# TalShor/SciLMM

Measured on NVIDIA B200. Metric: reml_iter_time, lower is better.
Workload: dtype f64

## Files before the change

### scilmm_b200/csrc/chol.cu

```cuda
#include <algorithm>
#include <cmath>
#include <cstring>
#include <map>
#include <memory>
#include <vector>

#include "common.h"
#include "dense_tiles.cuh"
#include "dense_tiles_tma.cuh"
#include "potrf_block.cuh"
#include "skinny_ops.cuh"
#include "symbolic.h"

namespace slmm {

static thread_local std::string g_last_error;
void set_last_error(const std::string& msg) { g_last_error = msg; }
const std::string& last_error() { return g_last_error; }
int64_t g_launch_count = 0;

constexpr int NBO = 1024;

struct PullItem { int32_t p, c0, c1, e0, e1; };
struct PullEntry { int64_t rel_off, src_off; int32_t rsc, ta, tb, pad; };
// ... 169 lines not shown

__global__ void logdet_kernel(const double* __restrict__ Lx, const int32_t* __restrict__ col2sn,
                              const int32_t* __restrict__ sn_first, const int32_t* __restrict__ sn_nrow,
                              const int64_t* __restrict__ sn_lptr, int n, double* __restrict__ partial) {
  __shared__ double sh[256];
  double acc = 0.0;
  for (int j = blockIdx.x * blockDim.x + threadIdx.x; j < n; j += gridDim.x * blockDim.x) {
    const int s = col2sn[j], c = j - sn_first[s];
    acc += log(Lx[sn_lptr[s] + (int64_t)c * ((sn_nrow[s] + 1) & ~1) + c]);
  }
  sh[threadIdx.x] = acc;
  __syncthreads();
  for (int o = 128; o > 0; o >>= 1) {
    if (threadIdx.x < o) sh[threadIdx.x] += sh[threadIdx.x + o];
    __syncthreads();
  }
  if (threadIdx.x == 0) partial[blockIdx.x] = sh[0];
}

struct Launch {
  enum Kind { POTRF, GEMM_BIG, GEMM_SMALL, PULL_MAT, PULL_VEC, PULL_MAT_BIG, INIT_W, REDUCE, EV_RECORD, EV_WAIT,
              SKINNY_F1, SKINNY_F2 ,
              GEMM_TMA  } kind;
  int64_t off;
  int32_t count;
  int32_t grid;
  int32_t child_parity;
  double flops;
  int64_t tile_off;
  int32_t stream;
  int64_t aux_off = 0;
};

static CUtensorMap encode_tmap(const double* base, uint64_t rows, uint64_t cols, uint64_t ld) {
  typedef CUresult (*EncodeFn)(CUtensorMap*, CUtensorMapDataType, cuuint32_t, void*, const cuuint64_t*, const cuuint64_t*,
                               const cuuint32_t*, const cuuint32_t*, CUtensorMapInterleave, CUtensorMapSwizzle,
                               CUtensorMapL2promotion, CUtensorMapFloatOOBfill);
  static EncodeFn fn = nullptr;
  if (!fn) {
    void* p = nullptr;
    cudaDriverEntryPointQueryResult q;
    CUDA_OK(cudaGetDriverEntryPoint("cuTensorMapEncodeTiled", &p, cudaEnableDefault, &q));
    if (!p || q != cudaDriverEntryPointSuccess) throw std::runtime_error("cuTensorMapEncodeTiled is not available");
    fn = (EncodeFn)p;
  }
  CUtensorMap m;
  const cuuint64_t gdim[2] = {rows, cols};
  const cuuint64_t gstride[1] = {ld * sizeof(double)};
  const cuuint32_t box[2] = {16, (cuuint32_t)TMA_KS};
  const cuuint32_t estr[2] = {1, 1};
  const CUresult rc = fn(&m, CU_TENSOR_MAP_DATA_TYPE_FLOAT64, 2, (void*)base, gdim, gstride, box, estr, CU_TENSOR_MAP_INTERLEAVE_NONE,
                         CU_TENSOR_MAP_SWIZZLE_128B, CU_TENSOR_MAP_L2_PROMOTION_L2_128B, CU_TENSOR_MAP_FLOAT_OOB_FILL_NONE);
  if (rc != CUDA_SUCCESS) throw std::runtime_error("cuTensorMapEncodeTiled failed (" + std::to_string((int)rc) + ")");
  return m;
}

constexpr int BIG_STAGES = 4, SMALL_STAGES = 4;
constexpr int BIG_SMEM = BIG_STAGES * 16 * (128 + 4) * 2 * 8 + 2 * BIG_STAGES * 8;
constexpr int SMALL_SMEM = SMALL_STAGES * 16 * (64 + 4) * 2 * 8 + 2 * SMALL_STAGES * 8;
constexpr int BIG_THREADS = 32 * (2 * 4 + NPW), SMALL_THREADS = 32 * (2 * 2 + NPW);

struct Schedule {
  std::vector<Launch> launches;
  std::vector<GemmOp> gemm;
  std::vector<PotrfOp> potrf;
  std::vector<PullItem> pull;
  std::vector<PullEntry> pull_entries;
  DevPtr<PullEntry> d_pull_entries;
  std::vector<ReduceOp> reduce;
  std::vector<CUtensorMap> tmaps;
  DevPtr<CUtensorMap> d_tmaps;
  std::vector<int32_t> tile_op;
  DevPtr<int32_t> d_tile_op;
  int nevents = 0;
  int64_t ws_size = 0;
  int64_t ws2_size = 0;
  DevPtr<double> d_ws;
  DevPtr<double> d_ws2;
  DevPtr<ReduceOp> d_reduce;
  DevPtr<GemmOp> d_gemm;
  DevPtr<PotrfOp> d_potrf;
  DevPtr<PullItem> d_pull;
  double flops = 0;
  GraphExec gexec[2];
  bool graph_failed = false;
  void upload() {
    if (ws_size > 0 || ws2_size > 0) {
      d_ws = dev_alloc<double>(ws_size);
      d_ws2 = dev_alloc<double>(ws2_size);
      for (GemmOp& op : gemm) {
        if (op.flags & GF_WS) { op.C = d_ws.get() + (int64_t)(intptr_t)op.C; op.flags &= ~GF_WS; }
        if (op.flags & GF_WS2) { op.C = d_ws2.get() + (int64_t)(intptr_t)op.C; op.flags &= ~GF_WS2; }
      }
      for (ReduceOp& r : reduce) {
        r.ws = ((r.flags & GF_WS2) ? d_ws2 : d_ws).get() + (int64_t)(intptr_t)r.ws;
        r.flags &= ~GF_WS2;
      }
    }
    d_reduce = dev_upload(reduce.data(), reduce.size());
    d_gemm = dev_upload(gemm.data(), gemm.size());
    d_potrf = dev_upload(potrf.data(), potrf.size());
    d_pull = dev_upload(pull.data(), pull.size());
    d_tile_op = dev_upload(tile_op.data(), tile_op.size());
    d_tmaps = dev_upload(tmaps.data(), tmaps.size());
    d_pull_entries = dev_upload(pull_entries.data(), pull_entries.size());
  }
  size_t device_bytes() const {
    return gemm.size() * sizeof(GemmOp) + potrf.size() * sizeof(PotrfOp) + pull.size() * sizeof(PullItem) +
           reduce.size() * sizeof(ReduceOp) + (size_t)(ws_size + ws2_size) * 8 + tile_op.size() * 4 + pull_entries.size() * sizeof(PullEntry);
  }
};

struct PhaseBuilder {
  std::vector<GemmOp> big, small, sk1, sk2;
  std::vector<GemmOp> tma;
  int skinny_mt = 0;
  int ws_id = 0;
  std::vector<PotrfOp> potrf;
  std::vector<ReduceOp> reduces;
  int64_t ws_used = 0;
  bool allow_split = true;
  static bool tma_ok(const GemmOp& op) {
    return op.a_si == 1 && op.b_sj == 1 && op.a_kidx == nullptr && !(op.flags & GF_TRIL_B) &&
           (op.a_sk % 2) == 0 && (op.b_sk % 2) == 0 && op.a_sk > 0 && op.b_sk > 0 && op.K >= 64;
  }
  void push(const GemmOp& op, bool small_tiles) {
    const bool tma_splits_inplace = op.C == op.A && op.N + (int)(((uintptr_t)op.B >> 3) & 1) > 128;
    if (small_tiles) small.push_back(op);
    else if (tma_ok(op) && !tma_splits_inplace) tma.push_back(op);
    else big.push_back(op);
  }
  template <typename Push>
  void split_k(const GemmOp& op, int S, int kc, Push push) {
    const int64_t mn = (int64_t)op.M * op.N;
    ReduceOp r;
    memset(&r, 0, sizeof(r));
    r.C = op.C; r.c_si = op.c_si; r.c_sj = op.c_sj; r.M = op.M; r.N = op.N; r.S = S;
    r.flags = (op.flags & (GF_ACCUM | GF_NEG)) | (ws_id ? GF_WS2 : 0);
    r.ws = (const double*)(intptr_t)ws_used;
    reduces.push_back(r);
    for (int c = 0; c < S; c++) {
      GemmOp part = op;
      const int k0 = c * kc;
      part.K = std::min(kc, op.K - k0);
      if (op.a_kidx) part.a_kidx = op.a_kidx + k0; else part.A = op.A + (int64_t)k0 * op.a_sk;
      part.B = op.B + (int64_t)k0 * op.b_sk;
      part.C = (double*)(intptr_t)(ws_used + (int64_t)c * mn);
      part.c_si = 1; part.c_sj = op.M;
      part.flags = (ws_id ? GF_WS2 : GF_WS) | (op.flags & GF_TRIL_B);
      part.pad = k0;
      push(part);
    }
    ws_used += (int64_t)S * mn;
  }
  bool add_skinny(const GemmOp& op) {
    if (skinny_mt <= 0 || op.M > skinny_mt || op.a_si != 1 || op.c_si != 1 || (op.flags & (GF_LOWER | GF_BIGTILE))) return false;
    const bool f1 = op.b_sj == 1 && op.a_kidx == nullptr;
    if (!f1 && op.b_sk != 1) return false;
    if (!f1 && (op.flags & GF_TRIL_B)) return false;
    std::vector<GemmOp>& dst = f1 ? sk1 : sk2;
    const int cols = f1 ? SK_F1_COLS : SK_F2_COLS, kmin = 64;
    const int64_t nj = (op.N + cols - 1) / cols;
    int S = 1;
    const int64_t target = f1 ? 148 * 8 : 148 * 4;
    const bool can_split = allow_split && op.C != op.A;
    if (can_split && nj < target) S = (int)std::min<int64_t>((target + nj - 1) / nj, std::max(1, op.K / kmin));
    if (!f1 && skinny_mt < 8) S = std::max(S, (op.K + SK_F2_KMAX - 1) / SK_F2_KMAX);
    if (S > 1 && !can_split) return false;
    int kc = op.K;
    if (S > 1) {
      kc = (((op.K + S - 1) / S) + 15) / 16 * 16;
      if (!f1 && skinny_mt < 8) kc = std::min(kc, SK_F2_KMAX);
      S = (op.K + kc - 1) / kc;
    }
    if (S <= 1) { GemmOp o = op; o.pad = 0; dst.push_back(o); }
    else split_k(op, S, kc, [&](const GemmOp& part) { dst.push_back(part); });
    return true;
  }
  void add(GemmOp op) {
    if (op.M <= 0 || op.N <= 0 || op.K <= 0) return;
    if (add_skinny(op)) return;
    const bool lower = op.flags & GF_LOWER;
    const int64_t tb = (int64_t)((op.M + 127) / 128) * ((op.N + 127) / 128);
    const int64_t ts = (int64_t)((op.M + 63) / 64) * ((op.N + 63) / 64);
    const bool force_big = op.flags & GF_BIGTILE;
    op.flags &= ~GF_BIGTILE;
    const bool small_tiles = !force_big && (!(op.M > 64 && op.N > 64) || (!lower && tb < 40 && op.K >= 128) ||
                                            (lower && tb <= 64));
    const int64_t tiles = small_tiles ? ts : tb;
    if (allow_split && !lower && (op.flags & GF_TRIL_B) && op.K >= 4096 && op.C != op.A && !small_tiles) {
      const int kc = 2048;
      const int S = (op.K + kc - 1) / kc;
      split_k(op, S, kc, [&](GemmOp part) { part.flags = (ws_id ? GF_WS2 : GF_WS) | GF_TRIL_B; push(part, false); });
      return;
    }
    if (allow_split && !lower && !(op.flags & GF_TRIL_B) && tiles <= 148 && op.K >= 256 && op.C != op.A) {
      int S = (int)std::min<int64_t>(std::min<int64_t>(64, op.K / 64), std::max<int64_t>(1, 148 / tiles));
      const int kc = S > 0 ? (((op.K + S - 1) / S) + 15) / 16 * 16 : op.K;
      S = (op.K + kc - 1) / kc;
      if (S >= 2) {
        op.flags &= ~GF_TRIL_B;
        split_k(op, S, kc, [&](GemmOp part) { part.pad = 0; part.flags = ws_id ? GF_WS2 : GF_WS; push(part, small_tiles); });
        return;
      }
    }
    push(op, small_tiles);
  }
  void flush(Schedule& sch, int stream = 0) {
    const size_t first_launch = sch.launches.size();
    if (!potrf.empty()) {
      double pf = 0;
      for (const PotrfOp& o : potrf) pf += 2.0 * o.nb * o.nb * o.nb / 3.0;
      sch.launches.push_back({Launch::POTRF, (int64_t)sch.potrf.size(), (int32_t)potrf.size(), (int32_t)potrf.size(), 0, pf});
      sch.potrf.insert(sch.potrf.end(), potrf.begin(), potrf.end());
    }
    for (int pass = 0; pass < 3; pass++) {
      std::vector<GemmOp>& v = pass == 0 ? tma : pass == 1 ? big : small;
      if (v.empty()) continue;
      const int T = pass == 2 ? 64 : 128;
      int64_t tiles = 0;
      double lf = 0;
      for (GemmOp& op : v) {
        int em = 0, en = 0;
        if (pass == 0) {
          em = (int)(((uintptr_t)op.A >> 3) & 1);
          en = (int)(((uintptr_t)op.B >> 3) & 1);
          op.pad = em | (en << 1);
        }
        op.tiles_m = (op.M + em + T - 1) / T;
        op.tiles_n = (op.N + en + T - 1) / T;
        op.tile_start = (int32_t)tiles;
        tiles += (int64_t)op.tiles_m * op.tiles_n;
        double f = 2.0 * op.M * op.N * op.K;
        if (op.flags & GF_TRIL_B) f = (double)op.M * op.N * op.K;
        if (op.flags & GF_LOWER) {
          const double nn = std::min(op.M, op.N);
          f = 2.0 * op.K * ((double)op.M * op.N - nn * (nn - 1) / 2.0);
        }
        sch.flops += f;
        lf += f;
      }
      if (tiles > 2000000000LL) throw std::runtime_error("too many tiles in one phase");
      const int64_t tile_off = (int64_t)sch.tile_op.size();
      sch.tile_op.resize(tile_off + tiles);
      for (size_t q = 0; q < v.size(); q++)
        std::fill(sch.tile_op.begin() + tile_off + v[q].tile_start,
                  sch.tile_op.begin() + tile_off + v[q].tile_start + (int64_t)v[q].tiles_m * v[q].tiles_n, (int32_t)q);
      if (pass == 0) {
        for (GemmOp& op : v) {
          const int sa = op.pad & 1, sb = (op.pad >> 1) & 1;
          sch.tmaps.push_back(encode_tmap(op.A - sa, (uint64_t)op.M + sa, (uint64_t)op.K, (uint64_t)op.a_sk));
          sch.tmaps.push_back(encode_tmap(op.B - sb, (uint64_t)op.N + sb, (uint64_t)op.K, (uint64_t)op.b_sk));
        }
      }
      Launch L{pass == 0 ? Launch::GEMM_TMA : pass == 1 ? Launch::GEMM_BIG : Launch::GEMM_SMALL, (int64_t)sch.gemm.size(),
               (int32_t)v.size(), (int32_t)tiles, 0, lf, tile_off};
      if (pass == 0) L.aux_off = (int64_t)sch.tmaps.size() - 2 * (int64_t)v.size();
      sch.launches.push_back(L);
      sch.gemm.insert(sch.gemm.end(), v.begin(), v.end());
    }
    for (int pass = 0; pass < 2; pass++) {
      std::vector<GemmOp>& v = pass == 0 ? sk1 : sk2;
      if (v.empty()) continue;
      const int T = pass == 0 ? SK_F1_COLS : SK_F2_COLS;
      int64_t tiles = 0;
      double lf = 0;
      for (GemmOp& op : v) {
        op.tiles_m = 1;
        op.tiles_n = (op.N + T - 1) / T;
        op.tile_start = (int32_t)tiles;
        tiles += op.tiles_n;
        const double f = (op.flags & GF_TRIL_B) ? (double)op.M * op.N * op.K : 2.0 * op.M * op.N * op.K;
        sch.flops += f;
        lf += f;
      }
      if (tiles > 2000000000LL) throw std::runtime_error("too many tiles in one phase");
      const int64_t tile_off = (int64_t)sch.tile_op.size();
      sch.tile_op.resize(tile_off + tiles);
      for (size_t q = 0; q < v.size(); q++)
        std::fill(sch.tile_op.begin() + tile_off + v[q].tile_start,
                  sch.tile_op.begin() + tile_off + v[q].tile_start + v[q].tiles_n, (int32_t)q);
      sch.launches.push_back({pass == 0 ? Launch::SKINNY_F1 : Launch::SKINNY_F2, (int64_t)sch.gemm.size(),
                              (int32_t)v.size(), (int32_t)tiles, skinny_mt, lf, tile_off});
      sch.gemm.insert(sch.gemm.end(), v.begin(), v.end());
    }
    if (!reduces.empty()) {
      int64_t blocks = 0;
      for (ReduceOp& r : reduces) {
        r.block_start = (int32_t)blocks;
        blocks += ((int64_t)r.M * r.N + 255) / 256;
      }
      sch.launches.push_back({Launch::REDUCE, (int64_t)sch.reduce.size(), (int32_t)reduces.size(), (int32_t)blocks, 0, 0.0});
      sch.reduce.insert(sch.reduce.end(), reduces.begin(), reduces.end());
      if (ws_id) sch.ws2_size = std::max(sch.ws2_size, ws_used); else sch.ws_size = std::max(sch.ws_size, ws_used);
    }
    for (size_t q = first_launch; q < sch.launches.size(); q++) sch.launches[q].stream = stream;
    big.clear(); small.clear(); tma.clear(); sk1.clear(); sk2.clear(); potrf.clear(); reduces.clear();
    ws_used = 0;
  }
  bool empty() const { return big.empty() && small.empty() && tma.empty() && sk1.empty() && sk2.empty() && potrf.empty(); }
};

static GemmOp make_op(double* C, int64_t c_si, int64_t c_sj, const double* A, int64_t a_si, int64_t a_sk,
                      const double* B, int64_t b_sj, int64_t b_sk, int M, int N, int K, int flags,
                      const int32_t* kidx = nullptr) {
  GemmOp op;
// ... 204 lines not shown
  if (nk == 0) return;
  if (!h->profiling) {
    const bool two = sch.nevents > 0 && h->s_main != nullptr && h->cur == nullptr;
    while ((int)h->events.size() < sch.nevents) h->events.push_back(make_event(cudaEventDisableTiming));
    const int gi = two ? 0 : 1;
    if (h->timeline && two) {
      while ((int)h->tl_events.size() < sch.nevents + 2) h->tl_events.push_back(make_event(cudaEventDefault));
      for (int q = 0; q < sch.nevents; q++) std::swap(h->events[q], h->tl_events[q + 2]);
      CUDA_OK(cudaEventRecord(h->tl_events[0].get(), 0));
      CUDA_OK(cudaStreamWaitEvent(h->s_main.get(), h->tl_events[0].get(), 0));
      CUDA_OK(cudaStreamWaitEvent(h->s_bulk.get(), h->tl_events[0].get(), 0));
      issue_schedule(h, sch, X, vec_arena, d_vptr, nrhs, true, nullptr, &h->tl_launch);
      CUDA_OK(cudaEventRecord(h->ev_join.get(), h->s_bulk.get()));
      CUDA_OK(cudaStreamWaitEvent(h->s_main.get(), h->ev_join.get(), 0));
      CUDA_OK(cudaEventRecord(h->tl_events[1].get(), h->s_main.get()));
      CUDA_OK(cudaStreamWaitEvent(0, h->tl_events[1].get(), 0));
      CUDA_OK(cudaEventSynchronize(h->tl_events[1].get()));
      for (int q = 0; q < sch.nevents; q++) std::swap(h->events[q], h->tl_events[q + 2]);
      h->tl_count = sch.nevents + 2;
      g_launch_count += nk;
      return;
    }
    const bool use_graph = !two && h->s_main != nullptr && !sch.graph_failed;
    if (use_graph && sch.gexec[gi] == nullptr) {
      try {
        sch.gexec[gi] = capture_schedule(h, sch, X, vec_arena, d_vptr, nrhs, two);
      } catch (const std::exception&) {
        sch.graph_failed = true;
      }
    }
    cudaGraphExec_t exec = (use_graph && !sch.graph_failed) ? sch.gexec[gi].get() : nullptr;
    if (exec != nullptr && h->cur != nullptr) {
      CUDA_OK(cudaGraphLaunch(exec, h->cur));
    } else if (exec != nullptr || two) {
      CUDA_OK(cudaEventRecord(h->ev_fork.get(), 0));
      CUDA_OK(cudaStreamWaitEvent(h->s_main.get(), h->ev_fork.get(), 0));
      if (exec != nullptr) {
        CUDA_OK(cudaGraphLaunch(exec, h->s_main.get()));
      } else {
        CUDA_OK(cudaStreamWaitEvent(h->s_bulk.get(), h->ev_fork.get(), 0));
        issue_schedule(h, sch, X, vec_arena, d_vptr, nrhs, true, nullptr);
        CUDA_OK(cudaEventRecord(h->ev_join.get(), h->s_bulk.get()));
        CUDA_OK(cudaStreamWaitEvent(h->s_main.get(), h->ev_join.get(), 0));
      }
      CUDA_OK(cudaEventRecord(h->ev_join.get(), h->s_main.get()));
      CUDA_OK(cudaStreamWaitEvent(0, h->ev_join.get(), 0));
    } else {
      issue_schedule(h, sch, X, vec_arena, d_vptr, nrhs, false, h->cur);
    }
  } else {
    const DevSym ds = h->devsym();
    cudaStream_t st = h->cur;
    std::vector<const Launch*> ks;
    for (const Launch& L : sch.launches) if (is_kernel(L)) ks.push_back(&L);
    const size_t nl = ks.size();
    std::vector<Event> ev(nl + 1);
    for (auto& e : ev) e = make_event(cudaEventDefault);
    CUDA_OK(cudaEventRecord(ev[0].get(), st));
    for (size_t i = 0; i < nl; i++) {
      launch_one(h, sch, *ks[i], ds, X, vec_arena, d_vptr, nrhs, st);
      CUDA_OK(cudaEventRecord(ev[i + 1].get(), st));
    }
    CUDA_OK(cudaEventSynchronize(ev[nl].get()));
    for (size_t i = 0; i < nl; i++) {
      float ms = 0;
      CUDA_OK(cudaEventElapsedTime(&ms, ev[i].get(), ev[i + 1].get()));
      const int k = (int)ks[i]->kind;
      h->prof_ms[k] += ms;
      h->prof_flops[k] += ks[i]->flops;
      h->prof_n[k] += 1;
      h->prof_launch_ms.push_back(ms);
      h->prof_launch_flops.push_back(ks[i]->flops);
      h->prof_launch_kind.push_back(k);
      h->prof_launch_grid.push_back((ks[i]->kind <= Launch::GEMM_SMALL || ks[i]->kind >= Launch::SKINNY_F1) ? ks[i]->grid : ks[i]->count);
    }
  }
  g_launch_count += nk;
  CUDA_OK(cudaGetLastError());
}

static void add_pull_items(Schedule& sch, const Symbolic& S, const std::vector<int64_t>& src_ptr, int level,
                           int lo_kind, Launch::Kind kind, int chunk, int min_rows = 0, int max_rows = 1 << 30) {
  const int64_t off = (int64_t)sch.pull.size();
  std::vector<std::vector<PullEntry>> per_item;
  for (int q = S.level_ptr[level]; q < S.level_ptr[level + 1]; q++) {
    const int p = S.level_sn[q];
    if (S.child_ptr[p + 1] == S.child_ptr[p]) continue;
    const int ns = S.sn_first[p + 1] - S.sn_first[p], ms = S.sn_nrow[p];
    if (ms < min_rows || ms >= max_rows) continue;
    const int a = lo_kind == 1 ? ns : 0, b = lo_kind == 0 ? ns : ms;
    std::vector<int> starts;
    for (int c0 = a; c0 < b;) {
      int c1 = std::min(b, c0 + chunk);
      if (c0 < ns && c1 > ns) c1 = ns;
      starts.push_back(c0);
      c0 = c1;
    }
    if (starts.empty()) continue;
    starts.push_back(b);
    const int nit = (int)starts.size() - 1;
    per_item.assign(nit, std::vector<PullEntry>());
    for (int cq = S.child_ptr[p]; cq < S.child_ptr[p + 1]; cq++) {
      const int c = S.child_idx[cq];
      const int nsc = S.sn_first[c + 1] - S.sn_first[c], rsc = S.sn_nrow[c] - nsc;
      if (rsc == 0) continue;
      const int64_t rel_off = S.sn_rowptr[c] + nsc;
      const int32_t* relc = S.rel.data() + rel_off;
      int t = (int)(std::lower_bound(relc, relc + rsc, a) - relc);
      int item = 0;
      while (t < rsc && relc[t] < b) {
        while (starts[item + 1] <= relc[t]) item++;
        int tb = t;
        while (tb < rsc && relc[tb] < starts[item + 1]) tb++;
        per_item[item].push_back({rel_off, src_ptr[c], rsc, t, tb, 0});
        t = tb;
      }
    }
    for (int i = 0; i < nit; i++) {
      if (per_item[i].empty()) continue;
      const int32_t e0 = (int32_t)sch.pull_entries.size();
      sch.pull_entries.insert(sch.pull_entries.end(), per_item[i].begin(), per_item[i].end());
      sch.pull.push_back({p, starts[i], starts[i + 1], e0, (int32_t)sch.pull_entries.size()});
    }
  }
  const int cnt = (int)(sch.pull.size() - off);
  if (cnt > 0) sch.launches.push_back({kind, off, cnt, 0, (level + 1) & 1, 0.0});
}

struct OuterBlock { int o0, nbo, ldw; double* winv; };
static int num_outer(int ns) { return (ns + NBO - 1) / NBO; }
static OuterBlock outer_block(const slmm_chol* h, int s, int ob) {
  const Symbolic& S = h->S;
  const int ns = S.sn_first[s + 1] - S.sn_first[s];
  OuterBlock b;
  b.o0 = ob * NBO;
  b.nbo = std::min(ns, b.o0 + NBO) - b.o0;
  if (b.nbo <= NBI) {
    b.winv = h->inv.get() + h->invptr[s] + (int64_t)(b.o0 / NBI) * NBI * NBI;
    b.ldw = NBI;
  } else {
    int64_t off = h->wptr[s];
    for (int q = 0; q < ob; q++) off += (int64_t)NBO * NBO;
    b.winv = h->W.get() + off;
    b.ldw = b.nbo;
  }
  return b;
}

struct FStep {
  enum Kind { POTRF, TRSM, UPD, WINV1, WINV2, CPANEL, OUTER, SCHUR } kind;
  int a, b;
};

static void build_factor_schedule(slmm_chol* h) {
  const Symbolic& S = h->S;
  Schedule& sch = h->fact;
  PhaseBuilder pb, pb_rest, pb_unrest;
  pb_rest.allow_split = pb_unrest.allow_split = false;
  int last_bulk_ev = -1, unrest_ev = -1;
  std::vector<std::vector<FStep>> prog;
  for (int d = S.nlevels - 1; d >= 0; d--) {
    add_pull_items(sch, S, h->uptr, d, 0, Launch::PULL_MAT, 8, 0, 512);
    add_pull_items(sch, S, h->uptr, d, 0, Launch::PULL_MAT_BIG, 4, 512);
    const int nl = S.level_ptr[d + 1] - S.level_ptr[d];
    prog.assign(nl, std::vector<FStep>());
    size_t max_steps = 0;
    for (int q = 0; q < nl; q++) {
      const int s = S.level_sn[S.level_ptr[d] + q];
      const int ns = S.sn_first[s + 1] - S.sn_first[s], ms = S.sn_nrow[s], rs = ms - ns;
      std::vector<FStep>& pr = prog[q];
      if (ns <= NBO) {
        const int nib = (ns + NBI - 1) / NBI;
        for (int ib = 0; ib < nib; ib++) {
          pr.push_back({FStep::POTRF, ib, 0});
          pr.push_back({FStep::TRSM, ib, 0});
          if (ib + 1 < nib) pr.push_back({FStep::UPD, ib, 0});
        }
        if (rs > 0) pr.push_back({FStep::SCHUR, 0, 0});
      } else {
        for (int ob = 0; ob < num_outer(ns); ob++) {
          const int o0 = ob * NBO, o1 = std::min(ns, o0 + NBO), w = o1 - o0;
          for (int c0 = o0; c0 < o1; c0 += NBI) {
            const int ib = c0 / NBI;
            pr.push_back({FStep::POTRF, ib, 0});
            if (std::min(o1, c0 + NBI) < o1) { pr.push_back({FStep::TRSM, ib, 0}); pr.push_back({FStep::UPD, ib, 0}); }
          }
          for (int m = NBI; m < w; m *= 2) { pr.push_back({FStep::WINV1, ob, m}); pr.push_back({FStep::WINV2, ob, m}); }
          if (ms > o1)
            for (int j = (w + 127) / 128 - 1; j >= 0; j--) pr.push_back({FStep::CPANEL, ob, j});
          if (o1 < ns) pr.push_back({FStep::OUTER, ob, 0});
          else if (rs > 0) pr.push_back({FStep::SCHUR, 0, 0});
        }
      }
      max_steps = std::max(max_steps, pr.size());
    }
    for (size_t ph = 0; ph < max_steps; ph++) {
      bool outer_done = false, needs_below = false;
      for (int q = 0; q < nl; q++) {
        if (ph >= prog[q].size()) continue;
        const FStep st = prog[q][ph];
        if (st.kind == FStep::CPANEL || st.kind == FStep::SCHUR) needs_below = true;
        const int s = S.level_sn[S.level_ptr[d] + q];
        const int f = S.sn_first[s], ns = S.sn_first[s + 1] - f, ms = S.sn_nrow[s], rs = ms - ns;
        const bool wide = ns > NBO;
        double* P = h->Lx.get() + S.sn_lptr[s];
        const int64_t ld = panel_ld(ms);
        if (st.kind == FStep::POTRF || st.kind == FStep::TRSM || st.kind == FStep::UPD) {
          const int ib = st.a, c0 = ib * NBI, c1 = std::min(ns, c0 + NBI), nb = c1 - c0;
          const int ob = c0 / NBO, ob0 = ob * NBO, ob_end = std::min(ns, ob0 + NBO);
          double* inv = h->inv.get() + h->invptr[s] + (int64_t)ib * NBI * NBI;
          int64_t inv_ld = NBI;
          if (wide) {
            const OuterBlock wb = outer_block(h, s, ob);
            if (wb.nbo > NBI) { inv = wb.winv + (c0 - ob0) + (int64_t)(c0 - ob0) * wb.ldw; inv_ld = wb.ldw; }
          }
          const int row_end = wide ? ob_end : ms;
          if (st.kind == FStep::POTRF) {
            pb.potrf.push_back({P + c0 + c0 * ld, inv, (int32_t)ld, nb, f + c0, (int32_t)inv_ld});
            sch.flops += (double)nb * nb * nb / 3.0;
          } else if (st.kind == FStep::TRSM) {
            pb.add(make_op(P + c1 + c0 * ld, 1, ld, P + c1 + c0 * ld, 1, ld, inv, 1, inv_ld, row_end - c1, nb, nb, 0));
          } else {
            pb.add(make_op(P + c1 + c1 * ld, 1, ld, P + c1 + c0 * ld, 1, ld, P + c1 + c0 * ld, 1, ld, row_end - c1,
                           ob_end - c1, nb, GF_LOWER | GF_ACCUM | GF_NEG));
          }
        } else if (st.kind == FStep::WINV1 || st.kind == FStep::WINV2) {
          const OuterBlock wb = outer_block(h, s, st.a);
          const int m = st.b, o0 = wb.o0;
          double* T = h->wscratch.get() + h->wscratch_off[s];
          int pair = 0;
          for (int lo = 0; lo + m < wb.nbo; lo += 2 * m, pair++) {
            const int m2 = std::min(m, wb.nbo - lo - m);
            double* Tp = T + (int64_t)pair * m * m;
            double* Ainv = wb.winv + lo + (int64_t)lo * wb.ldw;
            double* Binv = wb.winv + (lo + m) + (int64_t)(lo + m) * wb.ldw;
            double* X21 = wb.winv + (lo + m) + (int64_t)lo * wb.ldw;
            if (st.kind == FStep::WINV1)
              pb.add(make_op(Tp, 1, m2, P + (o0 + lo + m) + (int64_t)(o0 + lo) * ld, 1, ld, Ainv, wb.ldw, 1, m2, m, m, 0));
            else
              pb.add(make_op(X21, 1, wb.ldw, Binv, 1, wb.ldw, Tp, m2, 1, m2, m, m2, GF_NEG));
          }
        } else if (st.kind == FStep::CPANEL) {
          const OuterBlock wb = outer_block(h, s, st.a);
          const int o0 = wb.o0, o1 = o0 + wb.nbo, j0 = 128 * st.b, nj = std::min(128, wb.nbo - j0);
          const int K = std::min(wb.nbo, j0 + 128);
          pb.add(make_op(P + o1 + (int64_t)(o0 + j0) * ld, 1, ld, P + o1 + (int64_t)o0 * ld, 1, ld, wb.winv + j0, 1, wb.ldw,
                         ms - o1, nj, K, GF_BIGTILE));
        } else if (st.kind == FStep::OUTER) {
          const int ob0 = st.a * NBO, c1 = std::min(ns, ob0 + NBO);
          outer_done = true;
          const int nx = std::min(ns, c1 + NBO);
          const bool split = (ns - nx) >= NBO;
          const int ncols = split ? nx - c1 : ns - c1;
          const int below = ms - c1 - ncols;
          pb.add(make_op(P + c1 + c1 * ld, 1, ld, P + c1 + ob0 * ld, 1, ld, P + c1 + ob0 * ld, 1, ld, ncols,
                         ncols, c1 - ob0, GF_LOWER | GF_ACCUM | GF_NEG));
          if (below > 0)
            pb_unrest.add(make_op(P + (c1 + ncols) + c1 * ld, 1, ld, P + (c1 + ncols) + ob0 * ld, 1, ld, P + c1 + ob0 * ld, 1, ld,
                                  below, ncols, c1 - ob0, GF_ACCUM | GF_NEG));
          if (split)
            pb_rest.add(make_op(P + nx + nx * ld, 1, ld, P + nx + ob0 * ld, 1, ld, P + nx + ob0 * ld, 1, ld, ms - nx,
                                ns - nx, c1 - ob0, GF_LOWER | GF_ACCUM | GF_NEG));
        } else {
          double* U = h->arena[d & 1].get() + h->uptr[s];
          pb.add(make_op(U, 1, rs, P + ns, 1, ld, P + ns, 1, ld, rs, rs, ns, GF_LOWER | GF_NEG));
        }
      }
      const bool side = !pb_rest.empty() || !pb_unrest.empty();
      int ev_panel = -1;
      if (side) {
        ev_panel = sch.nevents++;
        sch.launches.push_back({Launch::EV_RECORD, 0, ev_panel, 0, 0, 0.0, 0, 0});
      }
      if (outer_done && last_bulk_ev >= 0) {
        sch.launches.push_back({Launch::EV_WAIT, 0, last_bulk_ev, 0, 0, 0.0, 0, 0});
        last_bulk_ev = -1;
      }
      if (needs_below && unrest_ev >= 0) {
        sch.launches.push_back({Launch::EV_WAIT, 0, unrest_ev, 0, 0, 0.0, 0, 0});
        unrest_ev = -1;
      }
      pb.flush(sch, 0);
      if (side) {
        sch.launches.push_back({Launch::EV_WAIT, 0, ev_panel, 0, 0, 0.0, 0, 1});
        if (!pb_unrest.empty()) {
          pb_unrest.flush(sch, 1);
          unrest_ev = sch.nevents++;
          sch.launches.push_back({Launch::EV_RECORD, 0, unrest_ev, 0, 0, 0.0, 0, 1});
          last_bulk_ev = unrest_ev;
        }
        if (!pb_rest.empty()) {
          pb_rest.flush(sch, 1);
          last_bulk_ev = sch.nevents++;
          sch.launches.push_back({Launch::EV_RECORD, 0, last_bulk_ev, 0, 0, 0.0, 0, 1});
        }
      }
    }
    if (last_bulk_ev >= 0) sch.launches.push_back({Launch::EV_WAIT, 0, last_bulk_ev, 0, 0, 0.0, 0, 0});
    last_bulk_ev = unrest_ev = -1;
    add_pull_items(sch, S, h->uptr, d, 1, Launch::PULL_MAT, 8, 0, 512);
    add_pull_items(sch, S, h->uptr, d, 1, Launch::PULL_MAT_BIG, 4, 512);
  }
  if (!h->wblocks.empty()) {
    sch.launches.push_back({Launch::INIT_W, 0, (int32_t)h->wblocks.size(), (int32_t)h->wblocks.size(), 0, 0.0});
    for (int t = 0; t < NBO / NBI; t++) {
      for (int half = 0; half < 2; half++) {
        for (int s2 = 0; s2 < S.nsuper; s2++) {
          const int ns = S.sn_first[s2 + 1] - S.sn_first[s2];
          if (ns <= NBI || ns > NBO) continue;
          double* P = h->Lx.get() + S.sn_lptr[s2];
          const int64_t ldp = panel_ld(S.sn_nrow[s2]);
          for (int ob = 0; ob < num_outer(ns); ob++) {
            const OuterBlock b = outer_block(h, s2, ob);
            if (b.nbo <= NBI || t * NBI >= b.nbo) continue;
            const int r0 = t * NBI, nbt = std::min(NBI, b.nbo - r0), ncols = std::min(b.nbo, r0 + NBI);
            double* inv64 = h->inv.get() + h->invptr[s2] + (int64_t)((b.o0 + r0) / NBI) * NBI * NBI;
            if (half == 0) {
              pb.add(make_op(b.winv + r0, 1, b.ldw, inv64, 1, NBI, b.winv + r0, b.ldw, 1, nbt, ncols, nbt, 0));
            } else if (r0 + nbt < b.nbo) {
              pb.add(make_op(b.winv + r0 + nbt, 1, b.ldw, P + (b.o0 + r0 + nbt) + (int64_t)(b.o0 + r0) * ldp, 1, ldp,
                             b.winv + r0, b.ldw, 1, b.nbo - r0 - nbt, ncols, nbt, GF_ACCUM | GF_NEG));
            }
          }
        }
        pb.flush(sch);
      }
    }
  }
  sch.upload();
}

static SolvePlan* get_plan(slmm_chol* h, int nrhs) {
  const int key = nrhs * 2 + (h->cur != nullptr ? 1 : 0);
  auto it = h->plans.find(key);
  if (it != h->plans.end()) return it->second.get();
  if (h->plans.size() >= 6) {
    CUDA_OK(cudaDeviceSynchronize());
    h->plans.clear();
  }
  const Symbolic& S = h->S;
  std::unique_ptr<SolvePlan> pl(new SolvePlan());
  pl->nrhs = nrhs;
  const int n = S.n;
  pl->X = dev_alloc<double>((size_t)n * nrhs);
  pl->X2 = dev_alloc<double>((size_t)n * nrhs);
  std::vector<int64_t> vptr(S.nsuper, 0);
  int64_t asz[2] = {0, 0};
  for (int d = 0; d < S.nlevels; d++) {
    int64_t off = 0;
    for (int q = S.level_ptr[d]; q < S.level_ptr[d + 1]; q++) {
      const int s = S.level_sn[q];
      vptr[s] = off;
      off += (int64_t)(S.sn_nrow[s] - (S.sn_first[s + 1] - S.sn_first[s])) * nrhs;
    }
    asz[d & 1] = std::max(asz[d & 1], off);
  }
  pl->arena[0] = dev_alloc<double>(asz[0]);
  pl->arena[1] = dev_alloc<double>(asz[1]);
  pl->d_vptr = dev_upload(vptr.data(), vptr.size());
  pl->bytes = ((size_t)2 * n * nrhs + asz[0] + asz[1]) * 8;
  const int64_t R = nrhs;
  PhaseBuilder pb, pb_rest;
  pb_rest.ws_id = 1;
  if (nrhs <= 32) pb.skinny_mt = nrhs <= 1 ? 1 : nrhs <= 2 ? 2 : nrhs <= 4 ? 4 : nrhs <= 8 ? 8 : nrhs <= 16 ? 16 : 32;
  const bool lookahead = nrhs >= 64;
  int last_bulk_ev = -1;
  auto flush_pair = [&](Schedule& sch, bool updated) {
    int ev_diag = -1;
    if (!pb_rest.empty()) {
      ev_diag = sch.nevents++;
      sch.launches.push_back({Launch::EV_RECORD, 0, ev_diag, 0, 0, 0.0, 0, 0});
    }
    if (updated && last_bulk_ev >= 0) {
      sch.launches.push_back({Launch::EV_WAIT, 0, last_bulk_ev, 0, 0, 0.0, 0, 0});
      last_bulk_ev = -1;
    }
    pb.flush(sch, 0);
    if (ev_diag >= 0) {
      sch.launches.push_back({Launch::EV_WAIT, 0, ev_diag, 0, 0, 0.0, 0, 1});
      pb_rest.flush(sch, 1);
      last_bulk_ev = sch.nevents++;
      sch.launches.push_back({Launch::EV_RECORD, 0, last_bulk_ev, 0, 0, 0.0, 0, 1});
    }
  };
  for (int d = S.nlevels - 1; d >= 0; d--) {
    add_pull_items(pl->fwd, S, vptr, d, 0, Launch::PULL_VEC, 4);
    int max_nob = 0;
    for (int q = S.level_ptr[d]; q < S.level_ptr[d + 1]; q++) {
      const int s = S.level_sn[q];
      max_nob = std::max(max_nob, num_outer(S.sn_first[s + 1] - S.sn_first[s]));
    }
    for (int ph = 0; ph < 2 * max_nob + 1; ph++) {
      bool updated = false;
      for (int q = S.level_ptr[d]; q < S.level_ptr[d + 1]; q++) {
        const int s = S.level_sn[q];
        const int f = S.sn_first[s], ns = S.sn_first[s + 1] - f, ms = S.sn_nrow[s], rs = ms - ns;
        const int nob = num_outer(ns);
        double* P = h->Lx.get() + S.sn_lptr[s];
        const int64_t ld = panel_ld(ms);
        double* Xs = pl->X.get() + (int64_t)f * R;
        double* Ys = pl->X2.get() + (int64_t)f * R;
        if (ph == 2 * nob) {
          if (rs > 0)
            pb.add(make_op(pl->arena[d & 1].get() + vptr[s], 1, R, Ys, 1, R, P + ns, 1, ld, nrhs, rs, ns, GF_NEG));
          continue;
        }
        if (ph > 2 * nob) continue;
        const OuterBlock b = outer_block(h, s, ph / 2);
        const int o1 = b.o0 + b.nbo;
        if (ph % 2 == 0) {
          pb.add(make_op(Ys + (int64_t)b.o0 * R, 1, R, Xs + (int64_t)b.o0 * R, 1, R, b.winv, 1, b.ldw, nrhs, b.nbo,
                         b.nbo, 0));
        } else if (o1 < ns) {
          updated = true;
          const int nx = std::min(ns, o1 + NBO);
          const bool split = lookahead && (ns - nx) >= NBO;
          pb.add(make_op(Xs + (int64_t)o1 * R, 1, R, Ys + (int64_t)b.o0 * R, 1, R, P + o1 + (int64_t)b.o0 * ld, 1, ld,
                         nrhs, (split ? nx : ns) - o1, b.nbo, GF_ACCUM | GF_NEG));
          if (split)
            pb_rest.add(make_op(Xs + (int64_t)nx * R, 1, R, Ys + (int64_t)b.o0 * R, 1, R, P + nx + (int64_t)b.o0 * ld, 1, ld,
                                nrhs, ns - nx, b.nbo, GF_ACCUM | GF_NEG));
        }
      }
      flush_pair(pl->fwd, updated);
    }
    if (last_bulk_ev >= 0) { pl->fwd.launches.push_back({Launch::EV_WAIT, 0, last_bulk_ev, 0, 0, 0.0, 0, 0}); last_bulk_ev = -1; }
    add_pull_items(pl->fwd, S, vptr, d, 1, Launch::PULL_VEC, 4);
  }
  for (int d = 0; d < S.nlevels; d++) {
    int max_nob = 0;
    for (int q = S.level_ptr[d]; q < S.level_ptr[d + 1]; q++) {
      const int s = S.level_sn[q];
      max_nob = std::max(max_nob, num_outer(S.sn_first[s + 1] - S.sn_first[s]));
    }
    for (int ph = 0; ph < 2 * max_nob + 1; ph++) {
      bool updated = false;
      for (int q = S.level_ptr[d]; q < S.level_ptr[d + 1]; q++) {
        const int s = S.level_sn[q];
        const int f = S.sn_first[s], ns = S.sn_first[s + 1] - f, ms = S.sn_nrow[s], rs = ms - ns;
        const int nob = num_outer(ns);
        double* P = h->Lx.get() + S.sn_lptr[s];
        const int64_t ld = panel_ld(ms);
        double* Xs = pl->X.get() + (int64_t)f * R;
        double* Ys = pl->X2.get() + (int64_t)f * R;
        if (ph == 0) {
          if (rs > 0)
            pb.add(make_op(Ys, 1, R, pl->X.get(), 1, R, P + ns, ld, 1, nrhs, ns, rs, GF_ACCUM | GF_NEG,
                           h->d_rows.get() + S.sn_rowptr[s] + ns));
          continue;
        }
        const int step = ph - 1, r = step / 2;
        if (r >= nob) continue;
        const OuterBlock b = outer_block(h, s, nob - 1 - r);
        if (step % 2 == 0) {
          pb.add(make_op(Xs + (int64_t)b.o0 * R, 1, R, Ys + (int64_t)b.o0 * R, 1, R, b.winv, b.ldw, 1, nrhs, b.nbo,
                         b.nbo, 0));
        } else if (b.o0 > 0) {
          updated = true;
          const int p0 = b.o0 - NBO;
          const bool split = lookahead && p0 >= NBO;
          const int lo = split ? p0 : 0;
          pb.add(make_op(Ys + (int64_t)lo * R, 1, R, Xs + (int64_t)b.o0 * R, 1, R, P + b.o0 + (int64_t)lo * ld, ld, 1, nrhs,
                         b.o0 - lo, b.nbo, GF_ACCUM | GF_NEG));
          if (split)
            pb_rest.add(make_op(Ys, 1, R, Xs + (int64_t)b.o0 * R, 1, R, P + b.o0, ld, 1, nrhs, p0, b.nbo,
                                GF_ACCUM | GF_NEG));
        }
      }
      flush_pair(pl->bwd, updated);
    }
    if (last_bulk_ev >= 0) { pl->bwd.launches.push_back({Launch::EV_WAIT, 0, last_bulk_ev, 0, 0, 0.0, 0, 0}); last_bulk_ev = -1; }
  }
  for (int d = S.nlevels - 1; d >= 0; d--) {
    for (int q = S.level_ptr[d]; q < S.level_ptr[d + 1]; q++) {
      const int s = S.level_sn[q];
      const int f = S.sn_first[s], ns = S.sn_first[s + 1] - f, ms = S.sn_nrow[s], rs = ms - ns;
      double* P = h->Lx.get() + S.sn_lptr[s];
      const int64_t ld = panel_ld(ms);
      pb.add(make_op(pl->X2.get() + (int64_t)f * R, 1, R, pl->X.get() + (int64_t)f * R, 1, R, P, 1, ld, nrhs, ns, ns, GF_TRIL_B));
      if (rs > 0)
        pb.add(make_op(pl->arena[d & 1].get() + vptr[s], 1, R, pl->X.get() + (int64_t)f * R, 1, R, P + ns, 1, ld, nrhs, rs, ns, 0));
// ... 565 lines not shown
```

Baseline: 0.1945.

## Split panel and trailing updates across streams to overlap the factorization critical path

Splits the CPANEL GEMM into a top strip needed by the next outer block, which stays on the main stream, and a lower remainder issued on the side stream. The unrestricted outer update is likewise split into a top chain part the next phase must wait on and a trailing part that can overlap. It also moves the narrow W-inverse construction so it runs during large root-level rest updates instead of after the factorization. The aim is to shorten the serial critical path of wide supernodes. The cost is more event records and waits, more kernel launches, and heuristic flop thresholds that may not fit other matrices.

```diff
diff --git a/scilmm_b200/csrc/chol.cu b/scilmm_b200/csrc/chol.cu
--- a/scilmm_b200/csrc/chol.cu
+++ b/scilmm_b200/csrc/chol.cu
@@ -345,6 +345,11 @@
       push(part);
     }
     ws_used += (int64_t)S * mn;
+  }
+  void add_panel(const GemmOp& op) {
+    if (op.M <= 0) return;
+    const bool to_tma = tma_ok(op) && op.N + (int)(((uintptr_t)op.B >> 3) & 1) <= 128;
+    split_k(op, 1, op.K, [&](const GemmOp& part) { (to_tma ? tma : big).push_back(part); });
   }
   bool add_skinny(const GemmOp& op) {
     if (skinny_mt <= 0 || op.M > skinny_mt || op.a_si != 1 || op.c_si != 1 || (op.flags & (GF_LOWER | GF_BIGTILE))) return false;
@@ -855,19 +860,64 @@
   int a, b;
 };
 
+static int chain_cols(int ns, int c1) {
+  const int nx = std::min(ns, c1 + NBO);
+  return (ns - nx) >= NBO ? nx - c1 : ns - c1;
+}
+static int chain_rows_end(int ns, int ms, int o0, int o1) {
+  if (o1 >= ns) return ms;
+  if (o0 >= NBO) {
+    const int c1 = o0, nx = std::min(ns, c1 + NBO), ncols = chain_cols(ns, c1);
+    const double nn = ns - nx;
+    double bulk = 2.0 * NBO * (double)(ms - c1 - ncols) * ncols;
+    if (ns - nx >= NBO) bulk += 2.0 * NBO * ((double)(ms - nx) * nn - nn * (nn - 1) / 2.0);
+    if (bulk > 6e10) return ms;
+  }
+  return o1 + chain_cols(ns, o1);
+}
+
 static void build_factor_schedule(slmm_chol* h) {
   const Symbolic& S = h->S;
   Schedule& sch = h->fact;
-  PhaseBuilder pb, pb_rest, pb_unrest;
-  pb_rest.allow_split = pb_unrest.allow_split = false;
-  int last_bulk_ev = -1, unrest_ev = -1;
+  PhaseBuilder pb, pb_panel, pb_unrest_top, pb_unrest, pb_rest;
+  pb_rest.allow_split = pb_unrest.allow_split = pb_unrest_top.allow_split = false;
+  pb_panel.ws_id = 1;
+  int last_bulk_ev = -1, top_ev = -1, tail_ev = -1;
+  bool narrow_w_done = h->wblocks.empty();
+  auto emit_narrow_w = [&]() {
+    sch.launches.push_back({Launch::INIT_W, 0, (int32_t)h->wblocks.size(), (int32_t)h->wblocks.size(), 0, 0.0});
+    for (int t = 0; t < NBO / NBI; t++) {
+      for (int half = 0; half < 2; half++) {
+        for (int s2 = 0; s2 < S.nsuper; s2++) {
+          const int ns = S.sn_first[s2 + 1] - S.sn_first[s2];
+          if (ns <= NBI || ns > NBO) continue;
+          double* P = h->Lx.get() + S.sn_lptr[s2];
+          const int64_t ldp = panel_ld(S.sn_nrow[s2]);
+          for (int ob = 0; ob < num_outer(ns); ob++) {
+            const OuterBlock b = outer_block(h, s2, ob);
+            if (b.nbo <= NBI || t * NBI >= b.nbo) continue;
+            const int r0 = t * NBI, nbt = std::min(NBI, b.nbo - r0), ncols = std::min(b.nbo, r0 + NBI);
+            double* inv64 = h->inv.get() + h->invptr[s2] + (int64_t)((b.o0 + r0) / NBI) * NBI * NBI;
+            if (half == 0) {
+              pb.add(make_op(b.winv + r0, 1, b.ldw, inv64, 1, NBI, b.winv + r0, b.ldw, 1, nbt, ncols, nbt, 0));
+            } else if (r0 + nbt < b.nbo) {
+              pb.add(make_op(b.winv + r0 + nbt, 1, b.ldw, P + (b.o0 + r0 + nbt) + (int64_t)(b.o0 + r0) * ldp, 1, ldp,
+                             b.winv + r0, b.ldw, 1, b.nbo - r0 - nbt, ncols, nbt, GF_ACCUM | GF_NEG));
+            }
+          }
+        }
+        pb.flush(sch);
+      }
+    }
+    narrow_w_done = true;
+  };
   std::vector<std::vector<FStep>> prog;
   for (int d = S.nlevels - 1; d >= 0; d--) {
     add_pull_items(sch, S, h->uptr, d, 0, Launch::PULL_MAT, 8, 0, 512);
     add_pull_items(sch, S, h->uptr, d, 0, Launch::PULL_MAT_BIG, 4, 512);
     const int nl = S.level_ptr[d + 1] - S.level_ptr[d];
     prog.assign(nl, std::vector<FStep>());
-    size_t max_steps = 0;
+    size_t max_steps = 0, narrow_steps = 0;
     for (int q = 0; q < nl; q++) {
       const int s = S.level_sn[S.level_ptr[d] + q];
       const int ns = S.sn_first[s + 1] - S.sn_first[s], ms = S.sn_nrow[s], rs = ms - ns;
@@ -889,16 +939,17 @@
             if (std::min(o1, c0 + NBI) < o1) { pr.push_back({FStep::TRSM, ib, 0}); pr.push_back({FStep::UPD, ib, 0}); }
           }
           for (int m = NBI; m < w; m *= 2) { pr.push_back({FStep::WINV1, ob, m}); pr.push_back({FStep::WINV2, ob, m}); }
-          if (ms > o1)
-            for (int j = (w + 127) / 128 - 1; j >= 0; j--) pr.push_back({FStep::CPANEL, ob, j});
+          if (ms > o1) pr.push_back({FStep::CPANEL, ob, 0});
           if (o1 < ns) pr.push_back({FStep::OUTER, ob, 0});
           else if (rs > 0) pr.push_back({FStep::SCHUR, 0, 0});
         }
       }
       max_steps = std::max(max_steps, pr.size());
+      if (ns <= NBO) narrow_steps = std::max(narrow_steps, pr.size());
     }
     for (size_t ph = 0; ph < max_steps; ph++) {
       bool outer_done = false, needs_below = false;
+      double rest_flops = 0;
       for (int q = 0; q < nl; q++) {
         if (ph >= prog[q].size()) continue;
         const FStep st = prog[q][ph];
@@ -945,31 +996,43 @@
           }
         } else if (st.kind == FStep::CPANEL) {
           const OuterBlock wb = outer_block(h, s, st.a);
-          const int o0 = wb.o0, o1 = o0 + wb.nbo, j0 = 128 * st.b, nj = std::min(128, wb.nbo - j0);
-          const int K = std::min(wb.nbo, j0 + 128);
-          pb.add(make_op(P + o1 + (int64_t)(o0 + j0) * ld, 1, ld, P + o1 + (int64_t)o0 * ld, 1, ld, wb.winv + j0, 1, wb.ldw,
-                         ms - o1, nj, K, GF_BIGTILE));
+          const int o0 = wb.o0, o1 = o0 + wb.nbo, t1 = chain_rows_end(ns, ms, o0, o1);
+          for (int j0 = 0; j0 < wb.nbo; j0 += 128) {
+            const int nj = std::min(128, wb.nbo - j0), K = std::min(wb.nbo, j0 + 128);
+            pb.add_panel(make_op(P + o1 + (int64_t)(o0 + j0) * ld, 1, ld, P + o1 + (int64_t)o0 * ld, 1, ld, wb.winv + j0, 1,
+                                 wb.ldw, t1 - o1, nj, K, 0));
+            pb_panel.add_panel(make_op(P + t1 + (int64_t)(o0 + j0) * ld, 1, ld, P + t1 + (int64_t)o0 * ld, 1, ld, wb.winv + j0,
+                                       1, wb.ldw, ms - t1, nj, K, 0));
+          }
         } else if (st.kind == FStep::OUTER) {
           const int ob0 = st.a * NBO, c1 = std::min(ns, ob0 + NBO);
           outer_done = true;
           const int nx = std::min(ns, c1 + NBO);
           const bool split = (ns - nx) >= NBO;
-          const int ncols = split ? nx - c1 : ns - c1;
-          const int below = ms - c1 - ncols;
+          const int ncols = chain_cols(ns, c1);
+          const int r0 = c1 + ncols, r1 = std::max(r0, chain_rows_end(ns, ms, c1, nx));
+          const int64_t tb = (int64_t)((ms - r0 + 127) / 128) * ((ncols + 127) / 128);
+          const bool big = ms - r0 > 64 && ncols > 64 && !(tb < 40 && c1 - ob0 >= 128);
           pb.add(make_op(P + c1 + c1 * ld, 1, ld, P + c1 + ob0 * ld, 1, ld, P + c1 + ob0 * ld, 1, ld, ncols,
                          ncols, c1 - ob0, GF_LOWER | GF_ACCUM | GF_NEG));
-          if (below > 0)
-            pb_unrest.add(make_op(P + (c1 + ncols) + c1 * ld, 1, ld, P + (c1 + ncols) + ob0 * ld, 1, ld, P + c1 + ob0 * ld, 1, ld,
-                                  below, ncols, c1 - ob0, GF_ACCUM | GF_NEG));
-          if (split)
+          auto unrest = [&](PhaseBuilder& dst, int a, int b) {
+            dst.add(make_op(P + a + c1 * ld, 1, ld, P + a + ob0 * ld, 1, ld, P + c1 + ob0 * ld, 1, ld, b - a, ncols,
+                            c1 - ob0, GF_ACCUM | GF_NEG | (big ? GF_BIGTILE : 0)));
+          };
+          unrest(pb_unrest_top, r0, r1);
+          unrest(pb_unrest, r1, ms);
+          if (split) {
+            const double nn = ns - nx;
+            rest_flops += 2.0 * (c1 - ob0) * ((double)(ms - nx) * nn - nn * (nn - 1) / 2.0);
             pb_rest.add(make_op(P + nx + nx * ld, 1, ld, P + nx + ob0 * ld, 1, ld, P + nx + ob0 * ld, 1, ld, ms - nx,
                                 ns - nx, c1 - ob0, GF_LOWER | GF_ACCUM | GF_NEG));
+          }
         } else {
           double* U = h->arena[d & 1].get() + h->uptr[s];
           pb.add(make_op(U, 1, rs, P + ns, 1, ld, P + ns, 1, ld, rs, rs, ns, GF_LOWER | GF_NEG));
         }
       }
-      const bool side = !pb_rest.empty() || !pb_unrest.empty();
+      const bool side = !pb_panel.empty() || !pb_unrest_top.empty() || !pb_unrest.empty() || !pb_rest.empty();
       int ev_panel = -1;
       if (side) {
         ev_panel = sch.nevents++;
@@ -979,57 +1042,37 @@
         sch.launches.push_back({Launch::EV_WAIT, 0, last_bulk_ev, 0, 0, 0.0, 0, 0});
         last_bulk_ev = -1;
       }
-      if (needs_below && unrest_ev >= 0) {
-        sch.launches.push_back({Launch::EV_WAIT, 0, unrest_ev, 0, 0, 0.0, 0, 0});
-        unrest_ev = -1;
+      if (needs_below && top_ev >= 0) {
+        sch.launches.push_back({Launch::EV_WAIT, 0, top_ev, 0, 0, 0.0, 0, 0});
+        top_ev = -1;
       }
       pb.flush(sch, 0);
       if (side) {
+        auto record = [&]() {
+          const int ev = sch.nevents++;
+          sch.launches.push_back({Launch::EV_RECORD, 0, ev, 0, 0, 0.0, 0, 1});
+          return ev;
+        };
         sch.launches.push_back({Launch::EV_WAIT, 0, ev_panel, 0, 0, 0.0, 0, 1});
-        if (!pb_unrest.empty()) {
-          pb_unrest.flush(sch, 1);
-          unrest_ev = sch.nevents++;
-          sch.launches.push_back({Launch::EV_RECORD, 0, unrest_ev, 0, 0, 0.0, 0, 1});
-          last_bulk_ev = unrest_ev;
+        pb_panel.flush(sch, 1);
+        if (!pb_unrest_top.empty()) {
+          pb_unrest_top.flush(sch, 1);
+          top_ev = record();
         }
-        if (!pb_rest.empty()) {
-          pb_rest.flush(sch, 1);
-          last_bulk_ev = sch.nevents++;
-          sch.launches.push_back({Launch::EV_RECORD, 0, last_bulk_ev, 0, 0, 0.0, 0, 1});
-        }
-      }
-    }
-    if (last_bulk_ev >= 0) sch.launches.push_back({Launch::EV_WAIT, 0, last_bulk_ev, 0, 0, 0.0, 0, 0});
-    last_bulk_ev = unrest_ev = -1;
+        const bool trailing = !pb_unrest.empty() || !pb_rest.empty();
+        pb_unrest.flush(sch, 1);
+        pb_rest.flush(sch, 1);
+        tail_ev = record();
+        if (trailing) last_bulk_ev = tail_ev;
+      }
+      if (d == 0 && !narrow_w_done && ph >= narrow_steps && rest_flops >= 1.5e11) emit_narrow_w();
+    }
+    if (tail_ev >= 0) sch.launches.push_back({Launch::EV_WAIT, 0, tail_ev, 0, 0, 0.0, 0, 0});
+    last_bulk_ev = top_ev = tail_ev = -1;
     add_pull_items(sch, S, h->uptr, d, 1, Launch::PULL_MAT, 8, 0, 512);
     add_pull_items(sch, S, h->uptr, d, 1, Launch::PULL_MAT_BIG, 4, 512);
   }
-  if (!h->wblocks.empty()) {
-    sch.launches.push_back({Launch::INIT_W, 0, (int32_t)h->wblocks.size(), (int32_t)h->wblocks.size(), 0, 0.0});
-    for (int t = 0; t < NBO / NBI; t++) {
-      for (int half = 0; half < 2; half++) {
-        for (int s2 = 0; s2 < S.nsuper; s2++) {
-          const int ns = S.sn_first[s2 + 1] - S.sn_first[s2];
-          if (ns <= NBI || ns > NBO) continue;
-          double* P = h->Lx.get() + S.sn_lptr[s2];
-          const int64_t ldp = panel_ld(S.sn_nrow[s2]);
-          for (int ob = 0; ob < num_outer(ns); ob++) {
-            const OuterBlock b = outer_block(h, s2, ob);
-            if (b.nbo <= NBI || t * NBI >= b.nbo) continue;
-            const int r0 = t * NBI, nbt = std::min(NBI, b.nbo - r0), ncols = std::min(b.nbo, r0 + NBI);
-            double* inv64 = h->inv.get() + h->invptr[s2] + (int64_t)((b.o0 + r0) / NBI) * NBI * NBI;
-            if (half == 0) {
-              pb.add(make_op(b.winv + r0, 1, b.ldw, inv64, 1, NBI, b.winv + r0, b.ldw, 1, nbt, ncols, nbt, 0));
-            } else if (r0 + nbt < b.nbo) {
-              pb.add(make_op(b.winv + r0 + nbt, 1, b.ldw, P + (b.o0 + r0 + nbt) + (int64_t)(b.o0 + r0) * ldp, 1, ldp,
-                             b.winv + r0, b.ldw, 1, b.nbo - r0 - nbt, ncols, nbt, GF_ACCUM | GF_NEG));
-            }
-          }
-        }
-        pb.flush(sch);
-      }
-    }
-  }
+  if (!narrow_w_done) emit_narrow_w();
   sch.upload();
 }
 
```

Result: no change. 0.1934, median of 6 (-0.6%).
